# johnnyjana730/MVIN

Measured on AMD Instinct MI355X. Metric: (user,item) pairs scored/sec @ dim=64 hop=2 fan-out=32; % HBM roofline, higher is better.
Workload: dtype f32

## Files before the change

mvin_amd/build.py:

```python
import argparse
import hashlib
import os
import shutil
import subprocess
import sys

PKG_DIR = os.path.dirname(os.path.abspath(__file__))
CSRC = os.path.join(PKG_DIR, "csrc")
INCLUDE = os.path.join(os.path.dirname(PKG_DIR), "include")
LIB_PATH = os.path.join(PKG_DIR, "libmvin_hip.so")
STAMP_PATH = LIB_PATH + ".stamp"
OBJ_DIR = os.path.join(PKG_DIR, "_build")
SOURCES = ["mvin_kernels.hip", "mvin_fused.hip", "mvin_fused_split.hip", "mvin_fused_packed.hip", "mvin_fused_wpp.hip", "mvin_fused_agg.hip", "mvin_fused_agg32.hip", "mvin_fused_wpp_fold.hip", "mvin_fused_d16.hip", "mvin_fused_d32.hip", "mvin_tail.hip", "mvin_tail_flash.hip", "mvin_score_small.hip", "mvin_keyaddr.hip", "mvin_keyaddr_stream.hip", "mvin_keyaddr_grouped.hip", "mvin_keyaddr_dense.hip", "mvin_keyaddr_static.hip", "mvin_keyaddr_flash.hip", "mvin_keyaddr_wave.hip", "mvin_hoist.hip", "mvin_probe.hip", "mvin_group.hip", "mvin_order.hip", "mvin_topk.hip", "mvin_rank.hip", "mvin_explore.hip", "mvin_ctr_metrics.hip", "mvin_prep.hip", "mvin_negatives.hip", "mvin_linear_mfma.hip", "mvin_bwd.hip", "mvin_abi.hip"]
HEADERS = ["mvin_common.h", "mvin_kernels.h", "mvin_fused_agg.h", "mvin_score_image.h", "mvin_row_select.h", "mvin_rnd.h"]
VERSION_SCRIPT = os.path.join(CSRC, "libmvin_hip.map")
ARCH = "gfx950"
FLAGS = ["-O3", "-std=c++17", "-fPIC", "-fvisibility=hidden", "-shared", f"--offload-arch={ARCH}"]


def _hipcc():
    for cand in (os.environ.get("HIPCC"), shutil.which("hipcc"), "/opt/rocm/bin/hipcc"):
        if cand and os.path.exists(cand):
            return cand
    raise RuntimeError("hipcc not found (looked at $HIPCC, PATH, /opt/rocm/bin/hipcc)")


def _existing(names, base):
    return [os.path.join(base, n) for n in names if os.path.exists(os.path.join(base, n))]


def _digest():
    h = hashlib.sha256(" ".join(FLAGS).encode())
    for path in _existing(SOURCES + HEADERS, CSRC) + [os.path.join(INCLUDE, "mvin_hip.h"), VERSION_SCRIPT]:
        with open(path, "rb") as f:
            h.update(path.encode())
            h.update(f.read())
    return h.hexdigest()


def needs_build():
    if not os.path.exists(LIB_PATH) or not os.path.exists(STAMP_PATH):
        return True
    with open(STAMP_PATH) as f:
        return f.read().strip() != _digest()


# ... 71 lines not shown
```

mvin_amd/csrc/mvin_abi.hip:

```cpp
#include <cstdlib>
#include <cstdarg>
#include <cstdio>
#include <string>

#include "mvin_kernels.h"
#include "mvin_fused_agg.h"

namespace {

thread_local std::string g_last_error;

int fail(int code, const char* fmt, ...) {
    char buf[512];
    va_list ap;
    va_start(ap, fmt);
    vsnprintf(buf, sizeof(buf), fmt, ap);
    va_end(ap);
    g_last_error = buf;
    return code;
}

int hip_result(hipError_t e, const char* what) {
    if (e == hipSuccess) return 0;
    fail((int)e, "%s: %s", what, hipGetErrorString(e));
    return (int)e;
}

bool bad_dim(int D) { return D < 4 || D > MVIN_MAX_DIM || (D & 3) != 0; }

size_t geom_sum(int B, int K, int from, int to) {
    size_t s = 0, p = 1;
    for (int e = 0; e <= to; ++e) {
        if (e >= from) s += p;
        p *= (size_t)K;
    }
    return s * (size_t)B;
}

}

extern "C" {

int mvin_abi_version(void) { return MVIN_ABI_VERSION; }

int mvin_debug_read_trace(long long* host_dst, size_t n) {
    if (!host_dst) return -1;
    static const bool ka = getenv("MVIN_KA_TRACE") != nullptr;
    static const bool pk = getenv("MVIN_PACK_TRACE") != nullptr;
    if (getenv("MVIN_SMALL_TRACE")) return (int)mvin::small_read_trace(host_dst, n);
    if (getenv("MVIN_KAF_TRACE")) return (int)mvin::kaf_read_trace(host_dst, n);
    if (pk) return (int)mvin::pack_read_prof(host_dst, n);
    if (ka && getenv("MVIN_KA_TRACE")[0] == '2') return (int)mvin::kas_read_trace(host_dst, n);
    return (int)(ka ? mvin::ka_read_trace(host_dst, n) : mvin::split_read_trace(host_dst, n));
}

const char* mvin_last_error(void) { return g_last_error.c_str(); }

size_t mvin_ent_elems(int B, int K, int levels) { return geom_sum(B, K, 0, levels); }

size_t mvin_rel_elems(int B, int K, int levels) { return levels > 0 ? geom_sum(B, K, 1, levels) : 0; }

int mvin_expand_ids(const int32_t* adj_entity, const int32_t* adj_relation, const int64_t* items_i64,
                    const int32_t* items_i32, int B, int K, int levels, int n_entity,
                    int32_t* ent_out, int32_t* rel_out, void* stream) {
    if (!ent_out || (!items_i64 && !items_i32) || (items_i64 && items_i32))
        return fail(-1, "mvin_expand_ids: need ent_out and exactly one of items_i64/items_i32");
    if (levels > 0 && (!adj_entity || !adj_relation || !rel_out))
        return fail(-1, "mvin_expand_ids: null adjacency/rel_out with levels=%d", levels);
    if (B <= 0 || K <= 0 || levels < 0 || n_entity <= 0)
// ... 494 lines not shown
    const float* b1c = Wv + (size_t)D * D;
    return gather_attn_l2_impl(ws, enc_entity, enc_relation, reinterpret_cast<const int32_t*>(parent_ids), parent_ids_i64 ? 2 : 1, t0, t1,
                               blk, Wv, b1c, b1c + D, q, blk, nullptr, B, parents_per_pair, K, D, n_entity, nR, nagg0, nagg1, nullptr,
                               nullptr, 0, stream, true, true, order, agg);
}

static bool fold_gather_applies(int D, int K, int n_entity, int nR, int64_t B);

static bool fold_applies(int D, int K, int n_entity, int nR, int64_t B) {
    if (D == 64) return agg_applies(D, K, n_entity, nR, B);
    static const char* e = getenv("MVIN_L2_AGG");
    if (e && e[0] == '0') return false;
    if (n_entity <= 0 || nR <= 0 || nR > 4096 || !mvin::fused_fold_supported(D, K)) return false;
    const uint64_t tb = (uint64_t)n_entity * (uint64_t)D * 4, ab = (uint64_t)n_entity * (uint64_t)K * 4;
    return tb < (1ull << 30) && ab < (1ull << 31) && n_entity <= (1 << 24) && (B <= 0 || (uint64_t)B * D * 4 < (1ull << 31)) &&
           mvin::fused_fold_lds_bytes(D, nR, K) <= 48 * 1024;
}

static size_t fold_blk_elems(int D) { return (size_t)12 * D * D + (size_t)3 * D; }

size_t mvin_fold_tables_elems(int n_entity, int D) {
    return n_entity > 0 && D > 0 ? (size_t)6 * n_entity * D + fold_blk_elems(D) : 0;
}

int mvin_score_l2_folded_supported(int D, int K, int n_entity, int nR) { return fold_applies(D, K, n_entity, nR, 1) ? 1 : 0; }

int mvin_fold_tables(const float* entity_emb, const int32_t* enc_entity, const int32_t* enc_relation, const float* t0, const float* W0,
                     const float* b0, const float* W1, const float* b1, const float* W2, const float* b2, const float* A0, const float* a0,
                     const float* Wmix, const float* bmix, const float* A1, int K, int D, int n_entity, int nR, float* ws, void* stream) {
    return mvin_fold_tables_ex(entity_emb, enc_entity, enc_relation, t0, W0, b0, W1, b1, W2, b2, A0, a0, Wmix, bmix, A1, 1, K, D, n_entity, nR, ws,
                               stream);
}

int mvin_fold_tables_ex(const float* entity_emb, const int32_t* enc_entity, const int32_t* enc_relation, const float* t0, const float* W0,
                        const float* b0, const float* W1, const float* b1, const float* W2, const float* b2, const float* A0, const float* a0,
                        const float* Wmix, const float* bmix, const float* A1, int aggregates, int K, int D, int n_entity, int nR, float* ws,
                        void* stream) {
    const char* who = "mvin_fold_tables";
    if (!entity_emb || !enc_entity || !enc_relation || !W0 || !W1 || !W2 || !A0 || !Wmix || !A1 || !ws) return fail(-1, "%s: null pointer", who);
    if (!(aggregates ? fold_applies(D, K, n_entity, nR, 1) : fold_gather_applies(D, K, n_entity, nR, 1)))
        return fail(-3, "%s: D = 64 with K in {16, 32, 64} or D = 32 with K in {16, 32}; n_entity <= 2^24, tables < 1 GiB, adjacency < 2 GiB, nR <= 4096 "
                        "(D=%d K=%d n_entity=%d nR=%d)", who, D, K, n_entity, nR);
    const size_t tab = (size_t)n_entity * D;
    float* blk = ws + 6 * tab;
    const float c = t0 ? 1.f / (float)K : 1.f;
    if (int rc = hip_result(mvin::launch_fold_prepare(W0, b0, W1, b1, W2, b2, A0, a0, Wmix, bmix, A1, c, D, blk, (hipStream_t)stream), who)) return rc;
    mvin_linear_args l{};
    l.src[0] = entity_emb;
    l.nsrc = 1;
    l.Dsrc = D;
    l.Dout = D;
    l.rows = n_entity;
    l.rows_per_group = 1;
    l.W = blk;
    l.w_zstride = (int64_t)D * D;
    l.out = ws;
    l.ldo = D;
    l.nz = 4;
    l.out_zstride = (int64_t)n_entity * D;
    if (int rc = mvin_linear_fwd(&l, stream)) return rc;
    if (!aggregates) return 0;
    mvin::EntityAggArgs f{};
    f.tabS = ws;
    f.selfS = ws + 2 * tab;
    f.tabG = ws + tab;
    f.selfG = ws;
    f.adj_e = enc_entity;
    f.adj_r = enc_relation;
    f.t0 = t0;
    f.outS = ws + 4 * tab;
    f.outG = ws + 5 * tab;
    f.n_entity = n_entity;
    f.K = K;
    f.D = D;
    f.nR = nR;
    f.table_bytes = (uint64_t)tab * 4;
    f.adj_bytes = (uint64_t)n_entity * (uint64_t)K * 4;
    return hip_result(mvin::launch_entity_aggregates(f, (hipStream_t)stream), who);
}

int mvin_score_l2_folded_fwd(const float* ws, const int32_t* enc_entity, const int32_t* enc_relation, const int64_t* items_i64,
                             const int32_t* items_i32, const float* t0, const float* t1, const float* q, const float* user_o, const float* A1,
                             const float* a1, const float* Wmix, int64_t B, int K, int D, int n_entity, int nR, float* out0, float* z2,
                             float* item_emb, float* scores, float* sig, void* stream) {
    const char* who = "mvin_score_l2_folded_fwd";
    if (!ws || !enc_entity || !enc_relation || !q || !user_o || !A1 || !Wmix || !scores) return fail(-1, "%s: null pointer", who);
    if ((items_i64 == nullptr) == (items_i32 == nullptr)) return fail(-1, "%s: exactly one of items_i64 / items_i32", who);
    if (B <= 0 || B >= (int64_t(1) << 31)) return fail(-2, "%s: B=%lld", who, (long long)B);
    if (!fold_applies(D, K, n_entity, nR, B)) return fail(-3, "%s: unsupported shape / sizes D=%d K=%d n_entity=%d nR=%d B=%lld", who, D, K, n_entity, nR, (long long)B);
    const size_t tab = (size_t)n_entity * D;
    const float* blk = ws + 6 * tab;
    const float* Wv = blk + (size_t)4 * D * D;
    const float* Wq = Wv + (size_t)D * D;
    const float* bv = Wq + (size_t)D * D;
    const float* bq = bv + D;
    const float* bm = bq + D;
    static const bool two = getenv("MVIN_L2_FOLD_TWO") && atoi(getenv("MVIN_L2_FOLD_TWO")) != 0;
    if (!two || D != 64)
    {
        const float* Wp = bm + D;
        const size_t DD = (size_t)D * D;
        return hip_result(mvin::launch_score_l2_folded(ws + 4 * tab, ws + 3 * tab, enc_entity, enc_relation,
                                                       items_i64 ? reinterpret_cast<const int32_t*>(items_i64) : items_i32, items_i64 ? 2 : 1, t1, q,
                                                       user_o, Wp, bq, Wp + DD, bv, Wp + 2 * DD, Wp + 3 * DD, a1, Wp + 4 * DD, Wp + 5 * DD, bm,
                                                       item_emb, scores, sig, B, K, D, nR, n_entity, (hipStream_t)stream),
                          who);
    }
    if (!out0 || !z2) return fail(-1, "%s: the two-launch variant (MVIN_L2_FOLD_TWO=1) needs the out0 / z2 scratch rows", who);
    mvin::FusedL2Args f{};
    f.table = ws;
    f.agg = const_cast<float*>(ws + 4 * tab);
// ... 262 lines not shown
                     const float* bmix, int64_t B, int D, int n_entity, float* item_emb, float* scores, float* sig,
                     int table_bf16, void* stream) {
    const char* who = "mvin_l2_tail_fwd";
    if (!mvin::l2_tail_supported(D)) return fail(-3, "%s: unsupported D=%d (16, 32, 64)", who, D);
    if (!entity_emb || !user_o || !nagg0 || !nagg1 || !A0 || !A1 || !Wmix || !scores) return fail(-1, "%s: null pointer", who);
    if ((items_i64 == nullptr) == (items_i32 == nullptr)) return fail(-1, "%s: exactly one of items_i64 / items_i32", who);
    if (W0 && !q) return fail(-1, "%s: the projection needs q", who);
    if (B <= 0 || n_entity <= 0) return fail(-2, "%s: bad sizes B=%lld n_entity=%d", who, (long long)B, n_entity);
    mvin::TailArgs t{};
    t.E = entity_emb;
    t.items64 = items_i64;
    t.items32 = items_i32;
    t.q = q;
    t.user_o = user_o;
    t.nagg0 = nagg0;
    t.nagg1 = nagg1;
    t.W0 = W0;
    t.b0 = b0;
    t.A0 = A0;
    t.a0 = a0;
    t.A1 = A1;
    t.a1 = a1;
    t.Wmix = Wmix;
    t.bmix = bmix;
    t.item_emb = item_emb;
    t.scores = scores;
    t.sig = sig;
    t.B = B;
    t.table_bf16 = table_bf16;
    t.n_entity = n_entity;
    return hip_result(mvin::launch_l2_tail(t, D, (hipStream_t)stream), who);
}

int mvin_score_l2_fwd(const mvin_score_l2_args* a, void* stream) {
    const char* who = "mvin_score_l2_fwd";
    if (!a) return fail(-1, "%s: null args", who);
    if (a->P < 1 || a->P > 8) return fail(-2, "%s: P=%d (1..8)", who, a->P);
    const bool grouped = a->uts && a->group_ws;
    if ((!a->V && !grouped) || !a->o_cat || !a->parents || !a->nagg0 || !a->nagg1 || !a->user_o || !a->scores || !a->items)
        return fail(-1, "%s: null workspace / output / items", who);
    if (a->uts && !a->users) return fail(-1, "%s: user_triplet_set given without user ids", who);
    if (a->group_ws && !a->uts) return fail(-1, "%s: group_ws is for the users feed (uts + users)", who);
    const int D = a->D, nR = a->n_relation;
    const int n_o = a->P + (a->h_set_w ? 1 : 0);
    mvin_linear_args l{};
    l.src[0] = reinterpret_cast<const float*>(a->entity_emb);
    l.ids[0] = reinterpret_cast<const int32_t*>(a->items);
    l.ids64 = 1;
    l.src_bf16 = a->table_bf16 ? 1 : 0;
    l.src_rows = a->n_entity;
    l.nsrc = 1;
    l.Dsrc = D;
    l.Dout = D;
    l.rows = a->B;
    l.W = a->relation_kge;
    l.rows_per_group = 1;
    l.out = a->V;
    l.ldo = (int64_t)nR * D;
    l.nz = nR;
    l.w_zstride = (int64_t)D * D;
    l.out_zstride = D;
    int rc = 0;
    bool flash = false;
    if (grouped) {
        int32_t* ws = a->group_ws;
        int32_t* seg_user = ws + 2 * (size_t)a->n_user + (size_t)a->B;
        int32_t* seg_ptr = seg_user + a->B;
        int32_t* nseg = seg_ptr + a->B + 2;
        int32_t* pair_index = nseg + 1;
        rc = mvin_group_pairs_by_user(a->users, nullptr, a->B, a->n_user, ws, seg_user, seg_ptr, nseg, pair_index, stream);
        if (rc) return rc;
        if (a->ka_flash && a->user_records && !a->table_bf16 && mvin::key_addr_flash_supported(D, a->P, a->Nm, nR, a->n_entity)) {
            rc = mvin_key_addressing_flash_prepare(reinterpret_cast<const float*>(a->entity_emb), a->relation_kge, a->h_set_w, a->user_mlp_W,
                                                   a->n_entity, nR, D, a->P, a->ka_flash, stream);
            if (rc) return rc;
            if (mvin_key_addressing_flash_ws_elems(a->B, a->n_user) > (size_t)2 * a->n_user + (size_t)a->B)
                return fail(-2, "%s: group_ws too small for the flash form's scheduling scratch", who);
            rc = mvin_key_addressing_flash_fwd(reinterpret_cast<const float*>(a->entity_emb), a->ka_flash, a->user_records, seg_user, seg_ptr,
                                               nseg, pair_index, a->items, nullptr, a->B, a->P, a->Nm, D, nR, a->n_entity, a->n_user,
                                               a->h_set_w != nullptr, a->user_mlp_b, a->user_o, ws, stream);
            flash = true;
        } else if (a->ka_er && a->user_records && !a->table_bf16 &&
            mvin_key_addressing_grouped_er_supported(D, a->P, a->Nm, nR, a->n_entity, a->h_set_w != nullptr)) {
            rc = mvin_project_relations(reinterpret_cast<const float*>(a->entity_emb), a->relation_kge, a->h_set_w, a->n_entity, nR, D,
                                        a->ka_er, stream);
            if (rc) return rc;
            rc = mvin_key_addressing_grouped_er_fwd(a->entity_emb, a->relation_kge, a->h_set_w, a->uts, a->user_records, a->ka_er, seg_user,
                                                    seg_ptr, nseg, pair_index, a->items, nullptr, (int)a->B, (int)a->B, a->P, a->Nm, D, nR,
                                                    a->n_entity, a->n_user, a->o_cat, (int64_t)n_o * D, stream);
        } else
        rc = mvin_key_addressing_grouped_rec_fwd(a->entity_emb, a->relation_kge, a->h_set_w, a->uts, a->user_records, seg_user, seg_ptr,
                                                 nseg, pair_index, a->items, nullptr, (int)a->B, (int)a->B, a->P, a->Nm, D, nR,
                                                 a->n_entity, a->n_user, a->o_cat, (int64_t)n_o * D, a->table_bf16, stream);
    } else {
        rc = mvin_linear_fwd(&l, stream);
        if (rc) return rc;
    }
    if (grouped) {
    } else if (a->uts)
        rc = mvin_key_addressing_users_fwd(a->entity_emb, a->V, a->h_set_w, a->uts, a->users, nullptr, a->P, (int)a->B, a->Nm,
                                           D, nR, a->n_entity, a->n_user, a->o_cat, (int64_t)n_o * D, a->table_bf16, stream);
    else
        rc = mvin_key_addressing_fwd(a->entity_emb, a->V, a->h_set_w, a->mem_h, a->mem_r, a->mem_t, a->P, (int)a->B, a->Nm, D,
                                     nR, a->n_entity, a->o_cat, (int64_t)n_o * D, a->table_bf16, stream);
    if (rc) return rc;
    if (!flash) {
    mvin_linear_args u{};
    u.src[0] = a->o_cat;
    u.nsrc = 1;
    u.Dsrc = n_o * D;
    u.Dout = D;
    u.rows = a->B;
    u.W = a->user_mlp_W;
    u.bias = a->user_mlp_b;
    u.rows_per_group = 1;
    u.out = a->user_o;
    u.ldo = D;
    u.nz = 1;
    rc = mvin_linear_fwd(&u, stream);
    if (rc) return rc;
    }
    if (a->fold_ws && a->fold_gather && a->enc_entity && a->enc_relation && a->W0 && a->W1 && a->W2 && !a->table_bf16 &&
        fold_gather_applies(D, a->K, a->n_entity, nR, a->B)) {
        rc = mvin_fold_tables_ex(reinterpret_cast<const float*>(a->entity_emb), a->enc_entity, a->enc_relation, a->t0, a->W0, a->b0, a->W1, a->b1,
                                 a->W2, a->b2, a->A0, a->a0, a->Wmix, a->bmix, a->A1, 0, a->K, D, a->n_entity, nR, a->fold_ws, stream);
        if (rc) return rc;
        const int32_t* order = nullptr;
        if (a->item_order_ws) {
            int32_t* ord = a->item_order_ws + mvin::order_ws_elems(a->B);
            rc = mvin_order_by_key(a->items, nullptr, a->B, a->item_order_ws, ord, stream);
            if (rc) return rc;
            order = ord;
        }
        return mvin_score_l2_folded_gather_fwd(a->fold_ws, a->enc_entity, a->enc_relation, a->items, nullptr, order, a->t0, a->t1, a->user_o,
                                               a->user_o, a->A1, a->a1, a->Wmix, a->B, a->K, D, a->n_entity, nR, a->item_emb, a->scores, a->sig,
                                               stream);
    }
    if (a->fold_ws && !a->fold_gather && a->enc_entity && a->enc_relation && a->W0 && a->W1 && a->W2 && !a->table_bf16 && fold_applies(D, a->K, a->n_entity, nR, a->B)) {
        rc = mvin_fold_tables(reinterpret_cast<const float*>(a->entity_emb), a->enc_entity, a->enc_relation, a->t0, a->W0, a->b0, a->W1, a->b1,
                              a->W2, a->b2, a->A0, a->a0, a->Wmix, a->bmix, a->A1, a->K, D, a->n_entity, nR, a->fold_ws, stream);
        if (rc) return rc;
        return mvin_score_l2_folded_fwd(a->fold_ws, a->enc_entity, a->enc_relation, a->items, nullptr, a->t0, a->t1, a->user_o, a->user_o, a->A1,
                                        a->a1, a->Wmix, a->B, a->K, D, a->n_entity, nR, a->nagg0, a->nagg1, a->item_emb, a->scores, a->sig,
                                        stream);
    }
    const bool enc = a->enc_entity && a->enc_relation && mvin::fused_packed_supported(D, a->K);
    const bool d32 = mvin::fused_d32_supported(D, a->K);
    if ((enc || d32) && a->prj_tables && a->W1 && !a->table_bf16 && prj_applies(D, a->K, enc, a->n_entity, nR, a->B)) {
        rc = mvin_project_tables(reinterpret_cast<const float*>(a->entity_emb), a->W1, a->W2, a->b1, a->b2, a->A0, a->a0,
                                 a->t0 != nullptr, a->K, a->n_entity, D, a->prj_tables, stream);
        if (rc) return rc;
        const int32_t* order = nullptr;
        if (enc && a->agg_tables && agg_applies(D, a->K, a->n_entity, nR, a->B)) {
            rc = mvin_entity_aggregates(a->prj_tables, a->enc_entity, a->enc_relation, a->t0, a->K, D, a->n_entity, nR, a->agg_tables, stream);
            if (rc) return rc;
            if (a->item_order_ws) {
                int32_t* ord = a->item_order_ws + mvin::order_ws_elems(a->B);
                rc = mvin_order_by_key(a->items, nullptr, a->B, a->item_order_ws, ord, stream);
                if (rc) return rc;
                order = ord;
            }
            rc = mvin_gather_attn_l2_agg_fwd(a->prj_tables, a->agg_tables, a->enc_entity, a->enc_relation, a->items, 1, order, a->t0, a->t1,
                                             a->user_o, (int)a->B, 1, a->K, D, a->n_entity, nR, a->nagg0, a->nagg1, stream);
        } else {
        if (enc && a->item_order_ws && mvin::fused_wpp_supported(D, a->K) && nR <= 4096) {
            mvin::FusedL2Args f{};
            f.prj = 1, f.K = a->K, f.nR = nR, f.P = a->B, f.parents_per_pair = 1, f.max_id = (unsigned)(a->n_entity - 1);
            f.table_bytes = (uint64_t)a->n_entity * D * 4, f.adj_bytes = (uint64_t)a->n_entity * a->K * 4;
            f.adj_r = a->enc_relation, f.W1 = a->W1, f.W2 = a->W2, f.q = a->user_o;
            if (mvin::fused_wpp_applies(f, D)) {
                int32_t* ord = a->item_order_ws + mvin::order_ws_elems(a->B);
                rc = mvin_order_by_key(a->items, nullptr, a->B, a->item_order_ws, ord, stream);
                if (rc) return rc;
// ... 113 lines not shown

int mvin_user_records_supported(int D, int P, int Nm, int nR, int table_bf16) {
    return !table_bf16 && mvin::key_addr_static_supported(D, P, Nm, nR) ? 1 : 0;
}

int mvin_build_user_records(const int32_t* uts, int n_user, int P, int Nm, int nR, int n_entity, int32_t* records, void* stream) {
    const char* who = "mvin_build_user_records";
    if (!uts || !records) return fail(-1, "%s: null pointer", who);
    if (n_user <= 0 || n_entity <= 0) return fail(-2, "%s: bad sizes n_user=%d n_entity=%d", who, n_user, n_entity);
    if (mvin::ka_rec_layout(P, Nm, nR).len == 0) return fail(-3, "%s: no record form for P=%d Nm=%d nR=%d (P 1..8, Nm 1..256, nR 1..4096)", who, P, Nm, nR);
    return hip_result(mvin::launch_user_records(uts, n_user, P, Nm, nR, n_entity, records, (hipStream_t)stream), who);
}

int mvin_key_addressing_grouped_fwd(const void* entity_emb, const float* relation_kge, const float* w,
                                    const int32_t* uts, const int32_t* seg_user, const int32_t* seg_ptr,
                                    const int32_t* nseg_dev, const int32_t* pair_index, const int64_t* items_i64,
                                    const int32_t* items_i32, int nseg, int B, int P, int Nm, int D, int nR,
                                    int n_entity, int n_user, float* out, int64_t ldo, int table_bf16, void* stream) {
    return mvin_key_addressing_grouped_rec_fwd(entity_emb, relation_kge, w, uts, nullptr, seg_user, seg_ptr, nseg_dev, pair_index, items_i64,
                                               items_i32, nseg, B, P, Nm, D, nR, n_entity, n_user, out, ldo, table_bf16, stream);
}

size_t mvin_project_relations_elems(int n_entity, int nR, int D) {
    if (n_entity <= 0 || nR <= 0 || D <= 0) return 0;
    return (size_t)nR * n_entity * D + (size_t)((n_entity + 3) & ~3) + (size_t)nR * D * D;
}

int mvin_project_relations(const float* entity_emb, const float* relation_kge, const float* w, int n_entity, int nR, int D, float* ws,
                           void* stream) {
    const char* who = "mvin_project_relations";
    if (!entity_emb || !relation_kge || !ws) return fail(-1, "%s: null pointer", who);
    if (n_entity <= 0 || nR <= 0 || (D != 16 && D != 32 && D != 64 && D != 128)) return fail(-2, "%s: n_entity=%d nR=%d D=%d", who, n_entity, nR, D);
    float* hs = ws + (size_t)nR * n_entity * D;
    float* RT = hs + (size_t)((n_entity + 3) & ~3);
    if (int rc = hip_result(mvin::launch_transpose_blocks(relation_kge, nR, D, RT, (hipStream_t)stream), who)) return rc;
    mvin_linear_args l{};
    l.src[0] = entity_emb;
    l.nsrc = 1;
    l.Dsrc = D;
    l.Dout = D;
    l.rows = n_entity;
    l.rows_per_group = 1;
    l.W = RT;
    l.w_zstride = (int64_t)D * D;
    l.out = ws;
    l.ldo = D;
    l.nz = nR;
    l.out_zstride = (int64_t)n_entity * D;
    if (int rc = mvin_linear_fwd(&l, stream)) return rc;
    if (w) return hip_result(mvin::launch_entity_dot(entity_emb, w, n_entity, D, hs, (hipStream_t)stream), who);
    return 0;
}

static int key_addressing_grouped_impl(const void* entity_emb, const float* relation_kge, const float* w,
                                        const int32_t* uts, const int32_t* user_records, const int32_t* seg_user,
                                        const int32_t* seg_ptr, const int32_t* nseg_dev, const int32_t* pair_index,
                                        const int64_t* items_i64, const int32_t* items_i32, int nseg, int B, int P, int Nm, int D,
                                        int nR, int n_entity, int n_user, float* out, int64_t ldo, int table_bf16, void* stream,
                                        const float* er_ws);

int mvin_key_addressing_flash_supported(int D, int P, int Nm, int nR, int n_entity) {
    return mvin::key_addr_flash_supported(D, P, Nm, nR, n_entity) ? 1 : 0;
}

static int flash_nseg_bound(int64_t B, int n_user) { return (int)(B < (int64_t)n_user ? B : (int64_t)n_user); }

size_t mvin_key_addressing_flash_ws_elems(int64_t B, int n_user) {
    if (B <= 0 || n_user <= 0) return 0;
    return mvin::key_addr_flash_ws_elems(B, flash_nseg_bound(B, n_user));
}

size_t mvin_key_addressing_flash_tables_elems(int n_entity, int nR, int D, int P, int has_set) {
    if (n_entity <= 0 || nR <= 0 || D <= 0 || P < 0) return 0;
    return mvin_project_relations_elems(n_entity, nR, D) + (size_t)(P + (has_set ? 1 : 0)) * n_entity * D;
}

int mvin_key_addressing_flash_prepare(const float* entity_emb, const float* relation_kge, const float* w, const float* user_mlp_W,
                                      int n_entity, int nR, int D, int P, float* ws, void* stream) {
    const char* who = "mvin_key_addressing_flash_prepare";
    if (!entity_emb || !relation_kge || !user_mlp_W || !ws) return fail(-1, "%s: null pointer", who);
    if (n_entity <= 0 || nR <= 0 || D != 64 || P < 1 || P > 8) return fail(-2, "%s: n_entity=%d nR=%d D=%d P=%d", who, n_entity, nR, D, P);
    if (int rc = mvin_project_relations(entity_emb, relation_kge, w, n_entity, nR, D, ws, stream)) return rc;
    mvin_linear_args l{};
    l.src[0] = entity_emb;
    l.nsrc = 1;
    l.Dsrc = D;
    l.Dout = D;
    l.rows = n_entity;
    l.rows_per_group = 1;
    l.W = user_mlp_W;
    l.w_zstride = (int64_t)D * D;
    l.out = ws + mvin_project_relations_elems(n_entity, nR, D);
    l.ldo = D;
    l.nz = P + (w ? 1 : 0);
    l.out_zstride = (int64_t)n_entity * D;
    return mvin_linear_fwd(&l, stream);
}

int mvin_key_addressing_flash_fwd(const float* entity_emb, const float* ws, const int32_t* user_records, const int32_t* seg_user,
                                  const int32_t* seg_ptr, const int32_t* nseg_dev, const int32_t* pair_index, const int64_t* items_i64,
                                  const int32_t* items_i32, int64_t B, int P, int Nm, int D, int nR, int n_entity, int n_user, int has_set,
                                  const float* user_mlp_b, float* user_o, int32_t* sched_ws, void* stream) {
    const char* who = "mvin_key_addressing_flash_fwd";
    if (!entity_emb || !ws || !user_records || !seg_user || !seg_ptr || !pair_index || !user_o || !sched_ws)
        return fail(-1, "%s: null pointer", who);
    if ((items_i64 == nullptr) == (items_i32 == nullptr)) return fail(-1, "%s: exactly one of items_i64 / items_i32", who);
    if (B <= 0 || B >= (int64_t(1) << 31) || n_user <= 0 || n_entity <= 0 || nR <= 0)
        return fail(-2, "%s: bad sizes B=%lld n_user=%d n_entity=%d nR=%d", who, (long long)B, n_user, n_entity, nR);
    if (!mvin::key_addr_flash_supported(D, P, Nm, nR, n_entity))
        return fail(-3, "%s: unsupported shape D=%d P=%d Nm=%d nR=%d n_entity=%d (D = 64, 1 <= P <= 8, Nm <= 64, nR * n_entity < 2^31)", who,
                    D, P, Nm, nR, n_entity);
    mvin::KaFlashArgs k{};
    k.E = entity_emb;
    k.ER = ws;
    k.hs = has_set ? ws + (size_t)nR * n_entity * D : nullptr;
    k.TW = ws + mvin_project_relations_elems(n_entity, nR, D);
    k.records = user_records;
    k.seg_user = seg_user;
    k.seg_ptr = seg_ptr;
    k.nseg_dev = nseg_dev;
    k.pair_index = pair_index;
    k.items64 = items_i64;
    k.items32 = items_i32;
    k.bmlp = user_mlp_b;
    k.user_o = user_o;
    k.P = P;
    k.Nm = Nm;
    k.nR = nR;
    k.n_entity = n_entity;
// ... 426 lines not shown
```

mvin_amd/csrc/mvin_kernels.h:

```cpp
#pragma once
#include <hip/hip_runtime.h>
#include <stdint.h>

#include "../../include/mvin_hip.h"
#include "mvin_common.h"

namespace mvin {

struct GatherAttnArgs {
    int gather;
    int table_bf16;
    const void* table;
    const int32_t* adj_e;
    const int32_t* adj_r;
    const int32_t* node_ids;
    const float* neigh;
    const int32_t* rel_ids;
    const float* rel_score;
    const float* self_vec;
    const float* Wc;
    const float* c_child;
    const float* Wagg;
    const float* bagg;
    float* out;
// ... 406 lines not shown
                           hipStream_t st);
hipError_t launch_kg_explore(const int64_t* eptr, const int32_t* edst, const int32_t* erel, int n_entity, int64_t M,
                             const int32_t* adj_entity, const int32_t* adj_relation, int K, const int32_t* seeds, int64_t n_seed,
                             int hops, void* ws, uint32_t* explored_bits, int64_t* out_counts, hipStream_t st);
size_t order_ws_elems(int64_t B);
hipError_t launch_order_by_key(const int64_t* k64, const int32_t* k32, int64_t B, int32_t* ws, int32_t* order, hipStream_t st);
bool fused_wpp_supported(int D, int K);
bool fused_wpp_applies(const FusedL2Args& a, int D);
hipError_t launch_gather_attn_l2_wpp(const FusedL2Args& a, hipStream_t st);
bool fused_agg_supported(int D, int K);
bool fused_fold_supported(int D, int K);
size_t fused_fold_lds_bytes(int D, int nR, int K);
bool fused_agg_applies(const FusedL2Args& a, int D);
hipError_t launch_entity_aggregates(const EntityAggArgs& a, hipStream_t st);
hipError_t launch_fold_prepare(const float* W0, const float* b0, const float* W1, const float* b1, const float* W2, const float* b2, const float* A0,
                               const float* a0, const float* Wmix, const float* bmix, const float* A1, float c, int D, float* blk, hipStream_t st);
hipError_t launch_l2_tail_fold(const TailFoldArgs& a, hipStream_t st);
hipError_t launch_score_l2_folded(const float* agg, const float* M0, const int32_t* adj_e, const int32_t* adj_r, const int32_t* items, int pid_stride,
                                  const float* t1, const float* q, const float* user_o, const float* Wq, const float* bq, const float* Wv,
                                  const float* bv, const float* Wqm, const float* A1, const float* a1, const float* Wm1, const float* Wm2,
                                  const float* bm, float* item_emb, float* scores, float* sig, int64_t B, int K, int D, int nR, int n_entity,
                                  hipStream_t st);
hipError_t launch_gather_attn_l2_agg(const FusedL2Args& a, hipStream_t st);
hipError_t launch_gather_attn_l2_d32(const FusedL2Args& a, int table_bf16, hipStream_t st, bool encoded = false);
bool fused_d16_supported(int D, int K);
bool fused_d16_applies(const FusedL2Args& a, int D);
hipError_t launch_gather_attn_l2_d16(const FusedL2Args& a, int table_bf16, hipStream_t st);
bool fused_l2_split_in_use();
hipError_t launch_gather_attn_l2_split(const FusedL2Args& a, int D, int table_bf16, hipStream_t st);
hipError_t split_read_trace(long long* host_dst, size_t n);
bool fused_packed_supported(int D, int K);
bool key_addr_static_er_ok(int P, int Nm, int nR, int n_entity, bool has_set);
hipError_t launch_transpose_blocks(const float* R, int nR, int D, float* RT, hipStream_t st);
hipError_t launch_entity_dot(const float* E, const float* w, int n, int D, float* out, hipStream_t st);
hipError_t launch_prj_prepare(const float* W1, const float* W2, const float* b1, const float* b2, const float* A0, const float* a0,
                              float c, int D, float* blk, hipStream_t st);
bool fused_packed_applies(const FusedL2Args& a, int D);
hipError_t pack_read_prof(long long* host_dst, size_t n);
hipError_t launch_gather_attn_l2_packed(const FusedL2Args& a, int D, int table_bf16, hipStream_t st);
hipError_t launch_encode_adjacency(const int32_t* adj_e, const int32_t* adj_r, int n_entity, int K, int32_t* cnt,
                                   int32_t* enc_e, int32_t* enc_r, hipStream_t st);
hipError_t ka_read_trace(long long* host_dst, size_t n);

}
```

Measured before the change: 493.1 million.

## Batch entity-table projections into one multi-job MFMA kernel for D=64

Adds a dedicated kernel that projects the entity embedding table through many 64x64 weight matrices in a single launch, with weights held in registers, a double-buffered row pipeline and MFMA f32 16x16x4. Relation projections, user-MLP tables and fold tables that were built by separate transpose and linear launches are now built as jobs of one or a few launches. When the key-addressing flash path and the fold path are both active, their table builds share one launch instead of being produced separately. The aim is to cut launch count and repeated reads of the entity table, at the cost of a new kernel whose job grid limit and per-wave register pressure may restrict occupancy.

```diff
diff --git a/mvin_amd/build.py b/mvin_amd/build.py
--- a/mvin_amd/build.py
+++ b/mvin_amd/build.py
@@ -11,7 +11,7 @@
 LIB_PATH = os.path.join(PKG_DIR, "libmvin_hip.so")
 STAMP_PATH = LIB_PATH + ".stamp"
 OBJ_DIR = os.path.join(PKG_DIR, "_build")
-SOURCES = ["mvin_kernels.hip", "mvin_fused.hip", "mvin_fused_split.hip", "mvin_fused_packed.hip", "mvin_fused_wpp.hip", "mvin_fused_agg.hip", "mvin_fused_agg32.hip", "mvin_fused_wpp_fold.hip", "mvin_fused_d16.hip", "mvin_fused_d32.hip", "mvin_tail.hip", "mvin_tail_flash.hip", "mvin_score_small.hip", "mvin_keyaddr.hip", "mvin_keyaddr_stream.hip", "mvin_keyaddr_grouped.hip", "mvin_keyaddr_dense.hip", "mvin_keyaddr_static.hip", "mvin_keyaddr_flash.hip", "mvin_keyaddr_wave.hip", "mvin_hoist.hip", "mvin_probe.hip", "mvin_group.hip", "mvin_order.hip", "mvin_topk.hip", "mvin_rank.hip", "mvin_explore.hip", "mvin_ctr_metrics.hip", "mvin_prep.hip", "mvin_negatives.hip", "mvin_linear_mfma.hip", "mvin_bwd.hip", "mvin_abi.hip"]
+SOURCES = ["mvin_kernels.hip", "mvin_fused.hip", "mvin_fused_split.hip", "mvin_fused_packed.hip", "mvin_fused_wpp.hip", "mvin_fused_agg.hip", "mvin_fused_agg32.hip", "mvin_fused_wpp_fold.hip", "mvin_fused_d16.hip", "mvin_fused_d32.hip", "mvin_tail.hip", "mvin_tail_flash.hip", "mvin_score_small.hip", "mvin_keyaddr.hip", "mvin_keyaddr_stream.hip", "mvin_keyaddr_grouped.hip", "mvin_keyaddr_dense.hip", "mvin_keyaddr_static.hip", "mvin_keyaddr_flash.hip", "mvin_keyaddr_wave.hip", "mvin_hoist.hip", "mvin_probe.hip", "mvin_group.hip", "mvin_order.hip", "mvin_topk.hip", "mvin_rank.hip", "mvin_explore.hip", "mvin_ctr_metrics.hip", "mvin_prep.hip", "mvin_negatives.hip", "mvin_linear_mfma.hip", "mvin_entity_tables.hip", "mvin_bwd.hip", "mvin_abi.hip"]
 HEADERS = ["mvin_common.h", "mvin_kernels.h", "mvin_fused_agg.h", "mvin_score_image.h", "mvin_row_select.h", "mvin_rnd.h"]
 VERSION_SCRIPT = os.path.join(CSRC, "libmvin_hip.map")
 ARCH = "gfx950"
diff --git a/mvin_amd/csrc/mvin_abi.hip b/mvin_amd/csrc/mvin_abi.hip
--- a/mvin_amd/csrc/mvin_abi.hip
+++ b/mvin_amd/csrc/mvin_abi.hip
@@ -35,6 +35,37 @@
         p *= (size_t)K;
     }
     return s * (size_t)B;
+}
+
+struct EntityTableList {
+    const float* E;
+    int n_entity;
+    hipStream_t st;
+    hipError_t err = hipSuccess;
+    int n = 0;
+    mvin::EntityTableJob jobs[mvin::kEtMaxJobs];
+    void add(const float* W, int w_nk, float* out) {
+        if (n == mvin::kEtMaxJobs) flush();
+        jobs[n++] = mvin::EntityTableJob{W, out, w_nk};
+    }
+    void flush() {
+        if (n > 0 && err == hipSuccess) err = mvin::launch_entity_tables(E, n_entity, jobs, n, st);
+        n = 0;
+    }
+};
+
+int build_entity_tables(const char* who, const float* E, int n_entity, const float* relation_kge, int nR, float* er, const float* user_mlp_W,
+                        int n_o, float* tw, const float* fold_blk, float* fold_tabs, void* stream) {
+    const size_t tab = (size_t)n_entity * 64, DD = (size_t)64 * 64;
+    EntityTableList l{E, n_entity, (hipStream_t)stream};
+    if (er)
+        for (int r = 0; r < nR; ++r) l.add(relation_kge + r * DD, 1, er + r * tab);
+    if (tw)
+        for (int j = 0; j < n_o; ++j) l.add(user_mlp_W + j * DD, 0, tw + j * tab);
+    if (fold_tabs)
+        for (int i = 0; i < 4; ++i) l.add(fold_blk + i * DD, 0, fold_tabs + i * tab);
+    l.flush();
+    return hip_result(l.err, who);
 }
 
 }
@@ -595,34 +626,27 @@
                                stream);
 }
 
-int mvin_fold_tables_ex(const float* entity_emb, const int32_t* enc_entity, const int32_t* enc_relation, const float* t0, const float* W0,
-                        const float* b0, const float* W1, const float* b1, const float* W2, const float* b2, const float* A0, const float* a0,
-                        const float* Wmix, const float* bmix, const float* A1, int aggregates, int K, int D, int n_entity, int nR, float* ws,
-                        void* stream) {
-    const char* who = "mvin_fold_tables";
+static int fold_tables_check(const char* who, const float* entity_emb, const int32_t* enc_entity, const int32_t* enc_relation, const float* W0,
+                             const float* W1, const float* W2, const float* A0, const float* Wmix, const float* A1, int aggregates, int K, int D,
+                             int n_entity, int nR, const float* ws) {
     if (!entity_emb || !enc_entity || !enc_relation || !W0 || !W1 || !W2 || !A0 || !Wmix || !A1 || !ws) return fail(-1, "%s: null pointer", who);
     if (!(aggregates ? fold_applies(D, K, n_entity, nR, 1) : fold_gather_applies(D, K, n_entity, nR, 1)))
         return fail(-3, "%s: D = 64 with K in {16, 32, 64} or D = 32 with K in {16, 32}; n_entity <= 2^24, tables < 1 GiB, adjacency < 2 GiB, nR <= 4096 "
                         "(D=%d K=%d n_entity=%d nR=%d)", who, D, K, n_entity, nR);
+    return 0;
+}
+
+static int fold_tables_block(const char* who, const float* t0, const float* W0, const float* b0, const float* W1, const float* b1, const float* W2,
+                             const float* b2, const float* A0, const float* a0, const float* Wmix, const float* bmix, const float* A1, int K, int D,
+                             int n_entity, float* ws, void* stream) {
+    const float c = t0 ? 1.f / (float)K : 1.f;
+    return hip_result(mvin::launch_fold_prepare(W0, b0, W1, b1, W2, b2, A0, a0, Wmix, bmix, A1, c, D, ws + (size_t)6 * n_entity * D,
+                                                (hipStream_t)stream), who);
+}
+
+static int fold_tables_aggregates(const char* who, const int32_t* enc_entity, const int32_t* enc_relation, const float* t0, int K, int D,
+                                  int n_entity, int nR, float* ws, void* stream) {
     const size_t tab = (size_t)n_entity * D;
-    float* blk = ws + 6 * tab;
-    const float c = t0 ? 1.f / (float)K : 1.f;
-    if (int rc = hip_result(mvin::launch_fold_prepare(W0, b0, W1, b1, W2, b2, A0, a0, Wmix, bmix, A1, c, D, blk, (hipStream_t)stream), who)) return rc;
-    mvin_linear_args l{};
-    l.src[0] = entity_emb;
-    l.nsrc = 1;
-    l.Dsrc = D;
-    l.Dout = D;
-    l.rows = n_entity;
-    l.rows_per_group = 1;
-    l.W = blk;
-    l.w_zstride = (int64_t)D * D;
-    l.out = ws;
-    l.ldo = D;
-    l.nz = 4;
-    l.out_zstride = (int64_t)n_entity * D;
-    if (int rc = mvin_linear_fwd(&l, stream)) return rc;
-    if (!aggregates) return 0;
     mvin::EntityAggArgs f{};
     f.tabS = ws;
     f.selfS = ws + 2 * tab;
@@ -640,6 +664,36 @@
     f.table_bytes = (uint64_t)tab * 4;
     f.adj_bytes = (uint64_t)n_entity * (uint64_t)K * 4;
     return hip_result(mvin::launch_entity_aggregates(f, (hipStream_t)stream), who);
+}
+
+int mvin_fold_tables_ex(const float* entity_emb, const int32_t* enc_entity, const int32_t* enc_relation, const float* t0, const float* W0,
+                        const float* b0, const float* W1, const float* b1, const float* W2, const float* b2, const float* A0, const float* a0,
+                        const float* Wmix, const float* bmix, const float* A1, int aggregates, int K, int D, int n_entity, int nR, float* ws,
+                        void* stream) {
+    const char* who = "mvin_fold_tables";
+    if (int rc = fold_tables_check(who, entity_emb, enc_entity, enc_relation, W0, W1, W2, A0, Wmix, A1, aggregates, K, D, n_entity, nR, ws)) return rc;
+    if (int rc = fold_tables_block(who, t0, W0, b0, W1, b1, W2, b2, A0, a0, Wmix, bmix, A1, K, D, n_entity, ws, stream)) return rc;
+    float* blk = ws + (size_t)6 * n_entity * D;
+    if (D == 64) {
+        if (int rc = build_entity_tables(who, entity_emb, n_entity, nullptr, 0, nullptr, nullptr, 0, nullptr, blk, ws, stream)) return rc;
+    } else {
+        mvin_linear_args l{};
+        l.src[0] = entity_emb;
+        l.nsrc = 1;
+        l.Dsrc = D;
+        l.Dout = D;
+        l.rows = n_entity;
+        l.rows_per_group = 1;
+        l.W = blk;
+        l.w_zstride = (int64_t)D * D;
+        l.out = ws;
+        l.ldo = D;
+        l.nz = 4;
+        l.out_zstride = (int64_t)n_entity * D;
+        if (int rc = mvin_linear_fwd(&l, stream)) return rc;
+    }
+    if (!aggregates) return 0;
+    return fold_tables_aggregates(who, enc_entity, enc_relation, t0, K, D, n_entity, nR, ws, stream);
 }
 
 int mvin_score_l2_folded_fwd(const float* ws, const int32_t* enc_entity, const int32_t* enc_relation, const int64_t* items_i64,
@@ -968,6 +1022,9 @@
     return hip_result(mvin::launch_l2_tail(t, D, (hipStream_t)stream), who);
 }
 
+static int flash_prepare_impl(const char* who, const float* entity_emb, const float* relation_kge, const float* w, const float* user_mlp_W,
+                              int n_entity, int nR, int D, int P, float* ws, float* fold_ws, void* stream);
+
 int mvin_score_l2_fwd(const mvin_score_l2_args* a, void* stream) {
     const char* who = "mvin_score_l2_fwd";
     if (!a) return fail(-1, "%s: null args", who);
@@ -998,6 +1055,10 @@
     l.out_zstride = D;
     int rc = 0;
     bool flash = false;
+    const bool fold_ok = a->fold_ws && a->enc_entity && a->enc_relation && a->W0 && a->W1 && a->W2 && !a->table_bf16;
+    const int fold_form = !fold_ok ? 0 : a->fold_gather ? (fold_gather_applies(D, a->K, a->n_entity, nR, a->B) ? 2 : 0)
+                                                        : (fold_applies(D, a->K, a->n_entity, nR, a->B) ? 1 : 0);
+    bool fold_built = false;
     if (grouped) {
         int32_t* ws = a->group_ws;
         int32_t* seg_user = ws + 2 * (size_t)a->n_user + (size_t)a->B;
@@ -1007,8 +1068,17 @@
         rc = mvin_group_pairs_by_user(a->users, nullptr, a->B, a->n_user, ws, seg_user, seg_ptr, nseg, pair_index, stream);
         if (rc) return rc;
         if (a->ka_flash && a->user_records && !a->table_bf16 && mvin::key_addr_flash_supported(D, a->P, a->Nm, nR, a->n_entity)) {
-            rc = mvin_key_addressing_flash_prepare(reinterpret_cast<const float*>(a->entity_emb), a->relation_kge, a->h_set_w, a->user_mlp_W,
-                                                   a->n_entity, nR, D, a->P, a->ka_flash, stream);
+            if (fold_form) {
+                rc = fold_tables_check("mvin_fold_tables", reinterpret_cast<const float*>(a->entity_emb), a->enc_entity, a->enc_relation, a->W0, a->W1,
+                                       a->W2, a->A0, a->Wmix, a->A1, fold_form == 1, a->K, D, a->n_entity, nR, a->fold_ws);
+                if (rc) return rc;
+                rc = fold_tables_block("mvin_fold_tables", a->t0, a->W0, a->b0, a->W1, a->b1, a->W2, a->b2, a->A0, a->a0, a->Wmix, a->bmix, a->A1,
+                                       a->K, D, a->n_entity, a->fold_ws, stream);
+                if (rc) return rc;
+                fold_built = true;
+            }
+            rc = flash_prepare_impl("mvin_key_addressing_flash_prepare", reinterpret_cast<const float*>(a->entity_emb), a->relation_kge, a->h_set_w,
+                                    a->user_mlp_W, a->n_entity, nR, D, a->P, a->ka_flash, fold_built ? a->fold_ws : nullptr, stream);
             if (rc) return rc;
             if (mvin_key_addressing_flash_ws_elems(a->B, a->n_user) > (size_t)2 * a->n_user + (size_t)a->B)
                 return fail(-2, "%s: group_ws too small for the flash form's scheduling scratch", who);
@@ -1056,10 +1126,10 @@
     rc = mvin_linear_fwd(&u, stream);
     if (rc) return rc;
     }
-    if (a->fold_ws && a->fold_gather && a->enc_entity && a->enc_relation && a->W0 && a->W1 && a->W2 && !a->table_bf16 &&
-        fold_gather_applies(D, a->K, a->n_entity, nR, a->B)) {
-        rc = mvin_fold_tables_ex(reinterpret_cast<const float*>(a->entity_emb), a->enc_entity, a->enc_relation, a->t0, a->W0, a->b0, a->W1, a->b1,
-                                 a->W2, a->b2, a->A0, a->a0, a->Wmix, a->bmix, a->A1, 0, a->K, D, a->n_entity, nR, a->fold_ws, stream);
+    if (fold_form == 2) {
+        if (!fold_built)
+            rc = mvin_fold_tables_ex(reinterpret_cast<const float*>(a->entity_emb), a->enc_entity, a->enc_relation, a->t0, a->W0, a->b0, a->W1, a->b1,
+                                     a->W2, a->b2, a->A0, a->a0, a->Wmix, a->bmix, a->A1, 0, a->K, D, a->n_entity, nR, a->fold_ws, stream);
         if (rc) return rc;
         const int32_t* order = nullptr;
         if (a->item_order_ws) {
@@ -1072,9 +1142,12 @@
                                                a->user_o, a->A1, a->a1, a->Wmix, a->B, a->K, D, a->n_entity, nR, a->item_emb, a->scores, a->sig,
                                                stream);
     }
-    if (a->fold_ws && !a->fold_gather && a->enc_entity && a->enc_relation && a->W0 && a->W1 && a->W2 && !a->table_bf16 && fold_applies(D, a->K, a->n_entity, nR, a->B)) {
-        rc = mvin_fold_tables(reinterpret_cast<const float*>(a->entity_emb), a->enc_entity, a->enc_relation, a->t0, a->W0, a->b0, a->W1, a->b1,
-                              a->W2, a->b2, a->A0, a->a0, a->Wmix, a->bmix, a->A1, a->K, D, a->n_entity, nR, a->fold_ws, stream);
+    if (fold_form == 1) {
+        if (fold_built)
+            rc = fold_tables_aggregates("mvin_fold_tables", a->enc_entity, a->enc_relation, a->t0, a->K, D, a->n_entity, nR, a->fold_ws, stream);
+        else
+            rc = mvin_fold_tables(reinterpret_cast<const float*>(a->entity_emb), a->enc_entity, a->enc_relation, a->t0, a->W0, a->b0, a->W1, a->b1,
+                                  a->W2, a->b2, a->A0, a->a0, a->Wmix, a->bmix, a->A1, a->K, D, a->n_entity, nR, a->fold_ws, stream);
         if (rc) return rc;
         return mvin_score_l2_folded_fwd(a->fold_ws, a->enc_entity, a->enc_relation, a->items, nullptr, a->t0, a->t1, a->user_o, a->user_o, a->A1,
                                         a->a1, a->Wmix, a->B, a->K, D, a->n_entity, nR, a->nagg0, a->nagg1, a->item_emb, a->scores, a->sig,
@@ -1254,22 +1327,26 @@
     if (!entity_emb || !relation_kge || !ws) return fail(-1, "%s: null pointer", who);
     if (n_entity <= 0 || nR <= 0 || (D != 16 && D != 32 && D != 64 && D != 128)) return fail(-2, "%s: n_entity=%d nR=%d D=%d", who, n_entity, nR, D);
     float* hs = ws + (size_t)nR * n_entity * D;
-    float* RT = hs + (size_t)((n_entity + 3) & ~3);
-    if (int rc = hip_result(mvin::launch_transpose_blocks(relation_kge, nR, D, RT, (hipStream_t)stream), who)) return rc;
-    mvin_linear_args l{};
-    l.src[0] = entity_emb;
-    l.nsrc = 1;
-    l.Dsrc = D;
-    l.Dout = D;
-    l.rows = n_entity;
-    l.rows_per_group = 1;
-    l.W = RT;
-    l.w_zstride = (int64_t)D * D;
-    l.out = ws;
-    l.ldo = D;
-    l.nz = nR;
-    l.out_zstride = (int64_t)n_entity * D;
-    if (int rc = mvin_linear_fwd(&l, stream)) return rc;
+    if (D == 64) {
+        if (int rc = build_entity_tables(who, entity_emb, n_entity, relation_kge, nR, ws, nullptr, 0, nullptr, nullptr, nullptr, stream)) return rc;
+    } else {
+        float* RT = hs + (size_t)((n_entity + 3) & ~3);
+        if (int rc = hip_result(mvin::launch_transpose_blocks(relation_kge, nR, D, RT, (hipStream_t)stream), who)) return rc;
+        mvin_linear_args l{};
+        l.src[0] = entity_emb;
+        l.nsrc = 1;
+        l.Dsrc = D;
+        l.Dout = D;
+        l.rows = n_entity;
+        l.rows_per_group = 1;
+        l.W = RT;
+        l.w_zstride = (int64_t)D * D;
+        l.out = ws;
+        l.ldo = D;
+        l.nz = nR;
+        l.out_zstride = (int64_t)n_entity * D;
+        if (int rc = mvin_linear_fwd(&l, stream)) return rc;
+    }
     if (w) return hip_result(mvin::launch_entity_dot(entity_emb, w, n_entity, D, hs, (hipStream_t)stream), who);
     return 0;
 }
@@ -1297,26 +1374,22 @@
     return mvin_project_relations_elems(n_entity, nR, D) + (size_t)(P + (has_set ? 1 : 0)) * n_entity * D;
 }
 
+static int flash_prepare_impl(const char* who, const float* entity_emb, const float* relation_kge, const float* w, const float* user_mlp_W,
+                              int n_entity, int nR, int D, int P, float* ws, float* fold_ws, void* stream) {
+    if (!entity_emb || !relation_kge || !user_mlp_W || !ws) return fail(-1, "%s: null pointer", who);
+    if (n_entity <= 0 || nR <= 0 || D != 64 || P < 1 || P > 8) return fail(-2, "%s: n_entity=%d nR=%d D=%d P=%d", who, n_entity, nR, D, P);
+    if (int rc = build_entity_tables(who, entity_emb, n_entity, relation_kge, nR, ws, user_mlp_W, P + (w ? 1 : 0),
+                                     ws + mvin_project_relations_elems(n_entity, nR, D), fold_ws ? fold_ws + (size_t)6 * n_entity * D : nullptr,
+                                     fold_ws, stream))
+        return rc;
+    if (w) return hip_result(mvin::launch_entity_dot(entity_emb, w, n_entity, D, ws + (size_t)nR * n_entity * D, (hipStream_t)stream), who);
+    return 0;
+}
+
 int mvin_key_addressing_flash_prepare(const float* entity_emb, const float* relation_kge, const float* w, const float* user_mlp_W,
                                       int n_entity, int nR, int D, int P, float* ws, void* stream) {
-    const char* who = "mvin_key_addressing_flash_prepare";
-    if (!entity_emb || !relation_kge || !user_mlp_W || !ws) return fail(-1, "%s: null pointer", who);
-    if (n_entity <= 0 || nR <= 0 || D != 64 || P < 1 || P > 8) return fail(-2, "%s: n_entity=%d nR=%d D=%d P=%d", who, n_entity, nR, D, P);
-    if (int rc = mvin_project_relations(entity_emb, relation_kge, w, n_entity, nR, D, ws, stream)) return rc;
-    mvin_linear_args l{};
-    l.src[0] = entity_emb;
-    l.nsrc = 1;
-    l.Dsrc = D;
-    l.Dout = D;
-    l.rows = n_entity;
-    l.rows_per_group = 1;
-    l.W = user_mlp_W;
-    l.w_zstride = (int64_t)D * D;
-    l.out = ws + mvin_project_relations_elems(n_entity, nR, D);
-    l.ldo = D;
-    l.nz = P + (w ? 1 : 0);
-    l.out_zstride = (int64_t)n_entity * D;
-    return mvin_linear_fwd(&l, stream);
+    return flash_prepare_impl("mvin_key_addressing_flash_prepare", entity_emb, relation_kge, w, user_mlp_W, n_entity, nR, D, P, ws, nullptr,
+                              stream);
 }
 
 int mvin_key_addressing_flash_fwd(const float* entity_emb, const float* ws, const int32_t* user_records, const int32_t* seg_user,
diff --git a/mvin_amd/csrc/mvin_entity_tables.hip b/mvin_amd/csrc/mvin_entity_tables.hip
--- /dev/null
+++ b/mvin_amd/csrc/mvin_entity_tables.hip
@@ -0,0 +1,133 @@
+#include "mvin_kernels.h"
+
+namespace mvin {
+
+typedef float f32x4 __attribute__((ext_vector_type(4)));
+
+constexpr int kEtD = 64;
+constexpr int kEtLd = 68;
+constexpr int kEtRows = 16;
+constexpr int kEtWgCap = 1024;
+
+struct EntityTableArgs {
+    const float* E;
+    int n_entity;
+    int njobs;
+    EntityTableJob jobs[kEtMaxJobs];
+};
+
+template <bool SMALL>
+__global__ __launch_bounds__(kBlock) __attribute__((amdgpu_waves_per_eu(4, 4))) void entity_tables_kernel(EntityTableArgs a) {
+    constexpr int D = kEtD, KS = D / 4, NT = D / 16;
+    __shared__ __attribute__((aligned(16))) float s_img[kBlock / 64][2][kEtRows * kEtLd];
+    const int lane = threadIdx.x & 63;
+    const int job = __builtin_amdgcn_readfirstlane((int)(blockIdx.y * (kBlock / 64) + (threadIdx.x >> 6)));
+    if (job >= a.njobs) return;
+    const int q16 = lane >> 4, l16 = lane & 15;
+    const float* __restrict__ W = a.jobs[job].W;
+    float* __restrict__ out = a.jobs[job].out;
+    const bool nk = a.jobs[job].w_nk != 0;
+
+    float aW[NT][KS];
+#pragma unroll
+    for (int nt = 0; nt < NT; ++nt) {
+        const int n = 16 * nt + l16;
+#pragma unroll
+        for (int s = 0; s < KS; ++s) aW[nt][s] = nk ? W[n * D + 4 * s + q16] : W[(4 * s + q16) * D + n];
+    }
+
+    const int64_t last = (int64_t)a.n_entity - 1;
+    const int ntiles = (int)(((int64_t)a.n_entity + kEtRows - 1) / kEtRows);
+    const int per = ntiles / (int)gridDim.x, rem = ntiles % (int)gridDim.x, bx = (int)blockIdx.x;
+    int tile = bx * per + (bx < rem ? bx : rem);
+    const int tend = tile + per + (bx < rem ? 1 : 0);
+    if (tile >= tend) return;
+    float* img = s_img[threadIdx.x >> 6][0];
+    float* oimg = s_img[threadIdx.x >> 6][1];
+    const int crow = lane >> 4, cc4 = 4 * (lane & 15);
+    auto tile_ptr = [&](const float* base, int t, int j) {
+        if constexpr (SMALL) {
+            const int64_t row = min((int64_t)t * kEtRows + 4 * j + crow, last);
+            return base + (size_t)row * D + cc4;
+        } else {
+            const int64_t row0 = min((int64_t)t * kEtRows, last - (kEtRows - 1));
+            return base + (size_t)row0 * D + (unsigned)((4 * j + crow) * D + cc4);
+        }
+    };
+    auto load_rows = [&](int t, f32x4 (&v)[NT]) {
+#pragma unroll
+        for (int j = 0; j < NT; ++j) v[j] = *reinterpret_cast<const f32x4*>(tile_ptr(a.E, t, j));
+    };
+    auto put_rows = [&](int t, int j) {
+        *reinterpret_cast<f32x4*>(const_cast<float*>(tile_ptr(out, t, j))) = *reinterpret_cast<const f32x4*>(oimg + (4 * j + crow) * kEtLd + cc4);
+    };
+    auto do_tile = [&](int t, auto first, const f32x4 (&cur)[NT], f32x4 (&nxt)[NT]) {
+        load_rows(t + 1 < tend ? t + 1 : t, nxt);
+        __builtin_amdgcn_sched_barrier(0);
+#pragma unroll
+        for (int j = 0; j < NT; ++j) *reinterpret_cast<f32x4*>(img + (4 * j + crow) * kEtLd + cc4) = cur[j];
+        __builtin_amdgcn_wave_barrier();
+        f32x4 acc[NT];
+#pragma unroll
+        for (int nt = 0; nt < NT; ++nt) acc[nt] = (f32x4){0.f, 0.f, 0.f, 0.f};
+#pragma unroll
+        for (int h = 0; h < 2; ++h) {
+            float b[KS / 2];
+#pragma unroll
+            for (int s = 0; s < KS / 2; ++s) b[s] = img[l16 * kEtLd + 4 * (s + h * (KS / 2)) + q16];
+#pragma unroll
+            for (int s = 0; s < KS / 2; ++s) {
+#pragma unroll
+                for (int nt = 0; nt < NT; ++nt)
+                    acc[nt] = __builtin_amdgcn_mfma_f32_16x16x4f32(aW[nt][s + h * (KS / 2)], b[s], acc[nt], 0, 0, 0);
+                if constexpr (!decltype(first)::value) if (s % 4 == 1) {
+                    put_rows(t - 1, (s + h * (KS / 2)) / 4);
+                    __builtin_amdgcn_sched_barrier(0);
+                }
+            }
+            __builtin_amdgcn_sched_barrier(0);
+        }
+        __builtin_amdgcn_wave_barrier();
+#pragma unroll
+        for (int nt = 0; nt < NT; ++nt) {
+            const f32x4 v = acc[nt] + 0.f;
+            *reinterpret_cast<f32x4*>(oimg + l16 * kEtLd + 16 * nt + 4 * q16) = v;
+        }
+        __builtin_amdgcn_wave_barrier();
+    };
+    f32x4 v0[NT], v1[NT];
+    load_rows(tile, v0);
+    do_tile(tile, std::true_type{}, v0, v1);
+    while (++tile < tend) {
+        do_tile(tile, std::false_type{}, v1, v0);
+        if (++tile >= tend) break;
+        do_tile(tile, std::false_type{}, v0, v1);
+    }
+#pragma unroll
+    for (int j = 0; j < NT; ++j) put_rows(tend - 1, j);
+}
+
+static int entity_tables_grid_x(int n_entity, int njobs) {
+    const int ngroups = (njobs + kBlock / 64 - 1) / (kBlock / 64);
+    const int64_t ntiles = ((int64_t)n_entity + kEtRows - 1) / kEtRows;
+    int64_t gx = kEtWgCap / (ngroups > 0 ? ngroups : 1);
+    if (gx > ntiles) gx = ntiles;
+    return (int)(gx < 1 ? 1 : gx);
+}
+
+hipError_t launch_entity_tables(const float* E, int n_entity, const EntityTableJob* jobs, int njobs, hipStream_t st) {
+    if (n_entity <= 0 || njobs < 1 || njobs > kEtMaxJobs) return hipErrorInvalidValue;
+    EntityTableArgs a{};
+    a.E = E;
+    a.n_entity = n_entity;
+    a.njobs = njobs;
+    for (int j = 0; j < njobs; ++j) a.jobs[j] = jobs[j];
+    const dim3 grid((unsigned)entity_tables_grid_x(n_entity, njobs), (unsigned)((njobs + kBlock / 64 - 1) / (kBlock / 64)));
+    if (n_entity < kEtRows)
+        entity_tables_kernel<true><<<grid, kBlock, 0, st>>>(a);
+    else
+        entity_tables_kernel<false><<<grid, kBlock, 0, st>>>(a);
+    return hipGetLastError();
+}
+
+}
diff --git a/mvin_amd/csrc/mvin_kernels.h b/mvin_amd/csrc/mvin_kernels.h
--- a/mvin_amd/csrc/mvin_kernels.h
+++ b/mvin_amd/csrc/mvin_kernels.h
@@ -462,6 +462,13 @@
 bool fused_packed_supported(int D, int K);
 bool key_addr_static_er_ok(int P, int Nm, int nR, int n_entity, bool has_set);
 hipError_t launch_transpose_blocks(const float* R, int nR, int D, float* RT, hipStream_t st);
+constexpr int kEtMaxJobs = 24;
+struct EntityTableJob {
+    const float* W;
+    float* out;
+    int w_nk;
+};
+hipError_t launch_entity_tables(const float* E, int n_entity, const EntityTableJob* jobs, int njobs, hipStream_t st);
 hipError_t launch_entity_dot(const float* E, const float* w, int n, int D, float* out, hipStream_t st);
 hipError_t launch_prj_prepare(const float* W1, const float* W2, const float* b1, const float* b2, const float* A0, const float* a0,
                               float c, int D, float* blk, hipStream_t st);
```

Measured after the change: 514.4 million, median of 6. +4.3%, better.
